# Da1yuqin/TCDiff

Measured on AMD Instinct MI355X. Metric: sampled clips/sec (3 dancers x 150 frames, 1000 DDPM steps), higher is better.
Workload: dtype bf16; 1 GPU; batch=16 clips/GPU, 3 dancers x 150 frames, 1000 DDPM steps (p_sample_loop, CFG w=2, cosine schedule), bf16, 1xMI355X; clips_per_gpu=16, ddpm_steps=1000

## Files before the change

### include/tcdiff_hip.h

```cpp
#ifndef TCDIFF_HIP_H
#define TCDIFF_HIP_H

#include <stdint.h>

#ifdef __cplusplus
extern "C" {
#endif

#ifndef __HIP__
typedef struct ihipStream_t* hipStream_t;
#endif

#define TCDIFF_OK 0
#define TCDIFF_ERR_ARG (-1)
#define TCDIFF_ERR_ALIGN (-2)
#define TCDIFF_ERR_LAUNCH (-3)
#define TCDIFF_ERR_UNSUPPORTED (-4)

#define TC_DTYPE_F32 0
#define TC_DTYPE_BF16 1
#define TC_DTYPE_BF16X3 2

#define TC_ACT_NONE 0
#define TC_ACT_RELU 1
// ... 130 lines not shown
    int film_ld;
    float ln_eps, n2_eps, n4_eps, nn_eps, scale_q;
    const float* filmb;
    const float* n3_g;
    const float* n3_b;
    const void* kf;
    const void* vf;
    int n_shared, nkt, Lk;
    int xres_rowmajor;
    int rope_rows;
    int dn;
    int mt;
    int out_ld;
    int nw;
    int seq_blocks;
    const void* sa_q;
    const void* sa_kf;
    const void* sa_vf;
    int sa_nkt;
    void* qf_out;
    void* kf_out;
    void* vf_out;
    int out_nkt;
} tcdiff_chain_args;

int tcdiff_chain(const tcdiff_chain_args* args, hipStream_t stream);

int tcdiff_chain_split(const tcdiff_chain_args* args, int part, const float* p_in, float* p_out, hipStream_t stream);

int tcdiff_pack_kv_frags(const void* Kc, const void* Vc, void* Kf, void* Vf, int n_slots, int H, int Lp, int nkt,
                         int key_lo, int key_hi, hipStream_t stream);

int tcdiff_attention(int dtype, const void* Q, const void* K, const void* V, void* O, int n_seq, int H, int Lq,
                     int Lk, int Lp_q, int Lp_k, int ldo, int n_shared, int ng, hipStream_t stream);

int tcdiff_ln_rot(int dtype, const float* x, int rows, const float* g, const float* b, float eps, void* h,
                  void* rot, float* y32, const float* rope, int pos_mod, int pos_base, hipStream_t stream);

int tcdiff_rope_table(const float* freqs, float* rope, int n_pos, hipStream_t stream);

int tcdiff_convert_pad(int dtype, const float* src, void* dst, int rows, int cols, int ld_dst, int rows_per_batch,
                       long batch_stride, long row_stride, hipStream_t stream);
int tcdiff_sinusoidal(int dtype, const int* times, int n, const float* freq, void* emb, hipStream_t stream);
int tcdiff_mean_pool(const float* x, float* out, int B, int S, int C, hipStream_t stream);
int tcdiff_add_act(int dtype, const float* a, const int* ia, const float* b, int n, int act, void* out,
                   float* out32, hipStream_t stream);
// ... 397 lines not shown
```

### tcdiff_amd/csrc/chain.hip

```cpp
#include "common.h"
#include "tcdiff_hip.h"

#include "chain_core.h"

#ifdef CH_ABLATE_ROWLAT
#define CH_RP_NEXT(rp, nt) do { } while (0)
#else
#define CH_RP_NEXT(rp, nt) rp_issue(rp, nt)
#endif

template <int HH, int MT, int NT, bool SELF = false>
DEVINL void cross_attention(const f32x4_t (&qacc)[NT][MT], const tcdiff_chain_args& a, int m0, int Mv, int lblk, char* abuf,
                            int wave, int lane) {
#ifdef CH_XATT_ONEPASS
    constexpr bool PARK = !SELF;
#else
    constexpr bool PARK = false;
#endif
    constexpr bool ONEPASS = SELF || PARK;
    constexpr int NPS = ONEPASS ? 1 : (MT == 4 ? 2 : 1), NML = ONEPASS ? MT : (MT == 1 ? 1 : 2);
    lane = fresh_v(lane);
    wave = fresh_s(wave) * (NT / 4) + HH;
    const int c = lane & 15, g = lane >> 4;
    const int M = Mv, L = a.L, nkt = SELF ? a.sa_nkt : a.nkt, Lk = SELF ? a.L : a.Lk;
    const float qs = a.scale_q * CH_LOG2E;
    u32x4 qf[MT][2];
// ... 159 lines not shown
                        pk.x = pack_bf2(o[dt][ml][0] * inv, o[dt][ml][1] * inv);
                        pk.y = pack_bf2(o[dt][ml][2] * inv, o[dt][ml][3] * inv);
                        *reinterpret_cast<uint2*>(abuf + wave * 8192 + act_wr_off(lane, dt) + mt * 2048) = pk;
                    }
                }
            }
        }
    }
}

#ifdef CH_STAMP
#ifndef CH_STAMP_BLOCK
#define CH_STAMP_BLOCK 0
#endif
#define CH_T(i) do { if (m0 == 64 * CH_STAMP_BLOCK && (threadIdx.x & 63) == 0 && (MODE == TC_CHAIN_B || MODE == TC_CHAIN_FULL)) \
        reinterpret_cast<unsigned long long*>(a.h_out)[(threadIdx.x >> 6) * 64 + (i)] = __builtin_amdgcn_s_memrealtime(); } while (0)
#define CH_TC(i) do { if (m0 == 64 * CH_STAMP_BLOCK && (threadIdx.x & 63) == 0 && (MODE == TC_CHAIN_B || MODE == TC_CHAIN_FULL)) \
        reinterpret_cast<unsigned long long*>(a.h_out)[(threadIdx.x >> 6) * 64 + (i)] = __builtin_amdgcn_s_memtime(); } while (0)
#else
#define CH_TC(i) do { } while (0)
#define CH_T(i) do { } while (0)
#endif

template <int MODE, int MT, int NT, int BRK>
DEVINL void chain_body(const tcdiff_chain_args& a) {
    constexpr int BR = BRK;
    constexpr int NW = ChW<NT>::NW, NTH = 64 * NW, RD = ChW<NT>::D;
    constexpr bool HAS_A = MODE == TC_CHAIN_A || MODE == TC_CHAIN_FULL || MODE == TC_CHAIN_FULL_LAST;
    constexpr bool FULL = MODE == TC_CHAIN_FULL || MODE == TC_CHAIN_FULL_LAST;
    constexpr bool LAST = MODE == TC_CHAIN_B_LAST || MODE == TC_CHAIN_FULL_LAST;
    constexpr bool FRONT = MODE == TC_CHAIN_FRONT;
    extern __shared__ __attribute__((aligned(16))) char smem[];
    const int tid = threadIdx.x, lane = tid & 63;
    const int wave = __builtin_amdgcn_readfirstlane(tid >> 6);
    const int c = lane & 15, g = lane >> 4;
    const int dn = FRONT ? a.dn : 1;
    const int dancer = FRONT ? (int)(blockIdx.x % (unsigned)dn) : 0;
    const int lblk = FRONT ? (int)(blockIdx.x / (unsigned)dn) : xcd_remap(blockIdx.x, gridDim.x);
    const bool seqcut = !FRONT && a.seq_blocks;
    const int nbs = seqcut ? (a.L + BR - 1) / BR : 1;
    const int bseq = seqcut ? lblk / nbs : 0, bis = seqcut ? lblk - bseq * nbs : 0;
    const int m0 = seqcut ? bseq * a.L + bis * BR : lblk * BR;
    CH_T(0);
    CH_TC(60);
    const int Mtot = a.M, L = a.L;
    const int M = seqcut ? (bseq + 1) * L : Mtot;
    char* abuf = smem + CH_ABUF;
// ... 80 lines not shown
            for (int kt = 0; kt < (FRONT ? 16 : 8); ++kt)
                stage_glds<16 * MT, NWL>(abuf + kt * 8192, reinterpret_cast<const char*>(a.A) + kt * TC_ROWB, FRONT ? 2048 : 1024, m0,
                                    M, a.a_mod, wave, lane);
        }
        ring_fill();
    }
    if (FRONT) {
        const float* const v[6] = {a.b3 + 512 * dancer, a.nn_g, a.nn_b, nullptr, nullptr, nullptr};
        store_consts(fetch_consts(nullptr, v));
    } else {
        const float* const v[6] = {nullptr, nullptr, a.n2_g, a.n2_b, nullptr, nullptr};
        store_consts(fetch_consts(a.film, v));
    }
    __builtin_amdgcn_s_waitcnt(0x0F70);
    __syncthreads();
    CH_T(1);


    float nmr[MT], rstd[MT];
    RowPipe<MT> rp;
    const long xrows = (long)Mtot * dn;
    const __amdgpu_buffer_rsrc_t xo = f32_buffer(a.xout, xrows * 512);
    Consts nxt;

    auto fc_epilogue = [&](float eps, int stamp) {
        CH_T(stamp);
        row_stats(acc, scr, wave, lane, eps, nmr, rstd);
        CH_T(stamp + 1);
        const int gg = fresh_v(g), wv = fresh_s(wave);
        const Rows rw = rows();
        const int cb0 = col_base_bytes<NT>(wv, gg);
        auto body = [&](int nt, int mt, const f32x4_t& G, const f32x4_t& Bv) {
            const f32x4_t x4 = rp.q[nt & 1][mt];
            f32x4_t o;
#pragma unroll
            for (int t = 0; t < 4; ++t) {
                float v = fmaf(fmaf(acc[nt][mt][t], rstd[mt], nmr[mt]), G[t], Bv[t]);
                v = x4[t] + v;
                acc[nt][mt][t] = v;
                o[t] = v;
            }
#ifdef CH_STORE_EARLY
            cb_store<NT>(xo, Mtot, wv, nt, rw.mc[mt], gg, o);
#endif
        };
        int fb[MT];
#pragma unroll
        for (int mt = 0; mt < MT; ++mt) {
            fb[mt] = rw.sidx[mt] * 4096 + cb0;
            asm volatile("" : "+v"(fb[mt]));
        }
#pragma unroll
        for (int nt = 0; nt < NT; ++nt) {
#pragma unroll
            for (int mt = 0; mt < MT; ++mt)
                body(nt, mt, lds4b(cfilm + fb[mt], 64 * nt), lds4b(cfilm + fb[mt], 2048 + 64 * nt));
            if (nt + 2 < NT) CH_RP_NEXT(rp, nt + 2);
            CH_FENCE();
        }
#ifndef CH_STORE_EARLY
#pragma unroll
        for (int nt = 0; nt < NT; ++nt)
#pragma unroll
            for (int mt = 0; mt < MT; ++mt) cb_store<NT>(xo, Mtot, wv, nt, rw.mc[mt], gg, acc[nt][mt]);
#endif
    };
    auto xres_start = [&]() {
        const Rows rw = rows();
        int rr[MT];
#pragma unroll
        for (int mt = 0; mt < MT; ++mt) rr[mt] = a.xres_mod > 0 ? rw.mc[mt] % a.xres_mod : rw.mc[mt];
        rp_start<NT>(rp, a.xres, rr, a.xres_rowmajor ? 0 : (a.xres_mod > 0 ? a.xres_mod : Mtot), a.xres_mod > 0 ? a.xres_mod : Mtot, wave,
                     fresh_v(g));
    };
    auto xout_start = [&]() {
        const Rows rw = rows();
        rp_start<NT>(rp, a.xout, rw.mc, Mtot, Mtot, wave, fresh_v(g));
    };
    auto rope_start = [&]() {
        const Rows rw = rows();
        int pos[MT];
        positions(rw, pos);
        rp_start<NT>(rp, a.rope, pos, a.rope_rows, a.rope_rows, wave, fresh_v(g));
    };

    if (HAS_A) {
        zero(acc);
        phase_n512<16, false, MT, NT>(acc, abuf, ws, lane);
        CH_T(2);
        xres_start();
        fc_epilogue(a.ln_eps, 40);
        CH_T(3);
        if (FULL) {
            const float* const v[6] = {nullptr, nullptr, n3_g, n3_b, nullptr, nullptr};
            nxt = fetch_consts(fcb_film, v);
        }
        rope_start();
        row_stats(acc, scr + 1024, wave, lane, a.n2_eps, nmr, rstd);
        CH_T(4);
        norm_to_lds<true, MT, NT>(acc, nmr, rstd, vecp(2), vecp(3), rp, abuf, wave, lane, nullptr);
        lds_barrier();
        CH_T(34);
        if (FULL) store_consts(nxt);
        zero(acc);
        if (!FULL) {
            phase_n512<16, false, MT, NT>(acc, abuf, ws, lane);
            store_heads<true, MT, NT>(acc, a.q_out, a.scale_q, L, a.Lp, a.H, m0, M, wave, lane, smem);
            return;
        }
#ifdef CH_STAMP
        {
            unsigned long long* sp = nullptr;
            if (m0 == 64 * CH_STAMP_BLOCK) {
                sp = reinterpret_cast<unsigned long long*>(a.h_out) + 512 + wave * 32;
                if (lane == 0) sp[16] = __builtin_amdgcn_s_memtime();
            }
            phase_n512<16, false, MT, NT>(acc, abuf, ws, lane, sp);
        }
#else
        phase_n512<16, false, MT, NT>(acc, abuf, ws, lane);
#endif
        CH_T(35);
        lds_barrier();
#ifndef CH_ABLATE_XATTN
        cross_attention<0>(acc, a, m0, M, lblk, abuf, wave, lane);
        if constexpr (NT == 8) cross_attention<1>(acc, a, m0, M, lblk, abuf, wave, lane);
#endif
        CH_T(36);
        lds_barrier();
    }
    if constexpr (!FRONT) {
    zero(acc);
    phase_n512<16, false, MT, NT>(acc, abuf, ws, lane);
    if (FULL)
        xout_start();
    else
        xres_start();
    CH_T(37);
    fc_epilogue(a.ln_eps, 42);
    CH_T(38);
    row_stats(acc, scr + 1024, wave, lane, a.n2_eps, nmr, rstd);
    CH_T(39);
    {
        const float* const v[6] = {a.b1, a.b1 + 512, nullptr, a.n4_g, a.n4_b, nullptr};
        nxt = fetch_consts(a.film3, v);
    }
    norm_to_lds<false, MT, NT>(acc, nmr, rstd, vecp(2), vecp(3), rp, abuf, wave, lane, nullptr);
    lds_barrier();
    store_consts(nxt);
    lds_barrier();
    CH_T(5);
    zero(acc);
#pragma unroll 1
    for (int ch = 0; ch < 4; ++ch) {
        f32x4_t a1[NT / 2][MT];
#pragma unroll
        for (int nt = 0; nt < NT / 2; ++nt)
#pragma unroll
            for (int mt = 0; mt < MT; ++mt) a1[nt][mt] = f32x4_t{0, 0, 0, 0};
        phase_ff1<MT, NT>(a1, abuf, ws, lane);
        CH_T(6 + 4 * ch);
        char* hb = h1c + (ch & 1) * 32768;
// ... 42 lines not shown
        }
#pragma unroll
        for (int nt = 0; nt < NT; ++nt) {
#pragma unroll
            for (int mt = 0; mt < MT; ++mt)
                body2(nt, mt, lds4b(cfilm + fb2[mt], 64 * nt), lds4b(cfilm + fb2[mt], 2048 + 64 * nt));
            if (nt + 2 < NT) CH_RP_NEXT(rp, nt + 2);
            CH_FENCE();
        }
    }
    CH_T(22);
    {
        const float* const v[6] = {a.b3, a.nn_g, a.nn_b, nullptr, nullptr, nullptr};
        nxt = fetch_consts(nullptr, v);
    }
    row_stats(acc, scr, wave, lane, a.n4_eps, nmr, rstd);
    CH_T(23);
    norm_to_lds<false, MT, NT>(acc, nmr, rstd, vecp(3), vecp(4), rp, abuf, wave, lane, nullptr);
    lds_barrier();
    store_consts(nxt);
    }
    CH_T(24);
    zero(acc);
    if (FRONT)
        phase_n512<32, false, MT, NT>(acc, abuf, ws, lane);
    else if (LAST)
        phase_n512<16, true, MT, NT>(acc, abuf, ws, lane);
    else
        phase_n512<16, false, MT, NT>(acc, abuf, ws, lane);
    CH_T(25);
    lds_barrier();
#ifndef CH_STORE_EARLY
    if (!LAST) rope_start();
#endif
    {
        const int g3 = fresh_v(g);
        const int cb3 = col_base_bytes<NT>(fresh_s(wave), g3);
        const Rows rw = rows();
#pragma unroll
        for (int nt = 0; nt < NT; ++nt) {
            const int n = 16 * NT * wave + 16 * nt + 4 * g3;
            const f32x4_t b4 = lds4b(vecp(0) + cb3, 64 * nt);
#pragma unroll
            for (int mt = 0; mt < MT; ++mt) {
                f32x4_t o;
#pragma unroll
                for (int t = 0; t < 4; ++t) {
                    acc[nt][mt][t] += b4[t];
                    o[t] = acc[nt][mt][t];
                }
                if (LAST && a.out_ld > 0) {
                    if (n < a.out_ld)
                        *reinterpret_cast<f32x4_t*>(reinterpret_cast<float*>(a.h_out) + (long)rw.mc[mt] * a.out_ld + n) = o;
                } else if (LAST) {
                    uint2 pk;
                    pk.x = pack_bf2(o[0], o[1]);
                    pk.y = pack_bf2(o[2], o[3]);
                    *reinterpret_cast<uint2*>(reinterpret_cast<uint16_t*>(a.h_out) + (long)rw.mc[mt] * 512 + n) = pk;
// ... 30 lines not shown
    if constexpr (FRAG) {
        if (frag_out) store_kfrag<MT>(acc, a.kf_out, bseq, bis * BR, a.out_nkt, wave, lane);
    }
    if (!frag_out) store_heads<false, MT, NT>(acc, a.k_out, 1.0f, L, a.Lp, a.H, m0, M, wave, lane, smem, dn, dancer);
    CH_T(31);
    zero(acc);
    if constexpr (FRAG) {
        if (frag_out) {
            phase_n512<16, true, MT, NT, true>(acc, smem + CH_ABUF2, ws, lane);
            CH_T(32);
            store_vfrag<MT>(acc, a.vf_out, bseq, bis * BR, a.out_nkt, L, wave, lane);
            CH_T(33);
            CH_TC(61);
            return;
        }
    }
    phase_n512<16, true, MT, NT>(acc, smem + CH_ABUF2, ws, lane);
    CH_T(32);
    store_heads<false, MT, NT>(acc, a.v_out, 1.0f, L, a.Lp, a.H, m0, M, wave, lane, smem, dn, dancer);
    CH_T(33);
    CH_TC(61);
}

template <int MODE, int MT, int NT>
__global__ __launch_bounds__(2048 / NT) void chain_kernel(tcdiff_chain_args a) {
    constexpr bool DUAL = (MODE == TC_CHAIN_FULL || MODE == TC_CHAIN_FULL_LAST) && NT == 4 && MT > 1;
    if constexpr (DUAL) {
        if (a.seq_blocks) {
            const int lblk = xcd_remap(blockIdx.x, gridDim.x);
            const int nbs = (a.L + 16 * MT - 1) / (16 * MT);
            if (a.L - (lblk % nbs) * 16 * MT <= 16) {
                chain_body<MODE, 1, NT, 16 * MT>(a);
                return;
            }
        }
    }
    chain_body<MODE, MT, NT, 16 * MT>(a);
}

static bool al16(const void* p) { return (reinterpret_cast<uintptr_t>(p) & 15) == 0; }

extern "C" int tcdiff_chain(const tcdiff_chain_args* a, hipStream_t stream) {
    if (!a || a->M <= 0 || a->L <= 0 || !a->A || !a->wstream) return TC_ERR_ARG;
    const bool front = a->mode == TC_CHAIN_FRONT;
    if (!front && a->L < 64) return TC_ERR_UNSUPPORTED;
    const int want = a->mode == TC_CHAIN_A ? 32 : a->mode == TC_CHAIN_B ? 144 : a->mode == TC_CHAIN_B_LAST ? 96 :
                     a->mode == TC_CHAIN_FULL ? 176 : a->mode == TC_CHAIN_FULL_LAST ? 128 : front ? 80 : -1;
    if (want < 0 || a->n_stages != want) return TC_ERR_ARG;
    if (a->out_ld < 0 || a->out_ld % 4 || a->out_ld > 512) return TC_ERR_ARG;
    const void* ptrs[] = {a->A, a->wstream, a->film, a->xres, a->xout, a->n2_g, a->n2_b, a->rope,
                          a->q_out, a->b1, a->film3, a->n4_g, a->n4_b, a->b3, a->nn_g, a->nn_b, a->k_out,
                          a->v_out, a->h_out, a->filmb, a->n3_g, a->n3_b, a->kf, a->vf};
    for (const void* p : ptrs)
        if (p && !al16(p)) return TC_ERR_ALIGN;
    if (front) {
        if (a->dn <= 0 || a->L % a->dn || a->L / a->dn < 8 || !a->b3 || !a->nn_g || !a->nn_b || !a->rope || !a->xout ||
            !a->q_out || !a->k_out || !a->v_out || a->H != 8 || a->Lp <= 0 || a->a_mod != 0)
            return TC_ERR_ARG;
        if ((long)a->M * 2048 >= (1L << 32)) return TC_ERR_ARG;
    } else {
// ... 8 lines not shown
    if (a->mode == TC_CHAIN_A && (!a->q_out || a->Lp <= 0)) return TC_ERR_ARG;
    if (has_b && (!a->b1 || !a->film3 || !a->n4_g || !a->n4_b || !a->b3)) return TC_ERR_ARG;
    const bool frag_out = a->qf_out || a->kf_out || a->vf_out;
    if (has_b && !last &&
        (!a->rope || !a->nn_g || !a->nn_b || (!frag_out && (!a->q_out || !a->k_out || !a->v_out)) || a->H != 8 || a->Lp <= 0))
        return TC_ERR_ARG;
    if (last && !a->h_out) return TC_ERR_ARG;
    if (full && (!a->filmb || !a->n3_g || !a->n3_b || !a->kf || !a->vf || a->nkt <= 0 ||
                 a->Lk <= 0 || a->Lk > 32 * a->nkt || a->n_shared < 0))
        return TC_ERR_ARG;
    if (a->seq_blocks && (front || a->M % a->L)) return TC_ERR_ARG;
    if (a->sa_q && (!full || !a->seq_blocks || !a->sa_kf || !a->sa_vf || a->sa_nkt <= 0 || a->L > 32 * a->sa_nkt)) return TC_ERR_ARG;
    if (frag_out && (!a->qf_out || !a->kf_out || !a->vf_out || !has_b || last || !a->seq_blocks || a->out_nkt <= 0 ||
                     a->L > 32 * a->out_nkt))
        return TC_ERR_ARG;
    if ((a->sa_q || frag_out) && a->nw == 4) return TC_ERR_UNSUPPORTED;
    for (const void* p : {a->sa_q, a->sa_kf, a->sa_vf, (const void*)a->qf_out, (const void*)a->kf_out, (const void*)a->vf_out})
        if (p && !al16(p)) return TC_ERR_ALIGN;
    if (a->sa_q && (long)(a->M / a->L) * 8 * a->sa_nkt * 4096 >= (1L << 32)) return TC_ERR_ARG;
    static tc_dev_state dev_state;
    const int n_cu = tc_device_once(dev_state, [](int) {
#define CH_FN(M_, NT_) reinterpret_cast<const void*>(chain_kernel<M_, 4, NT_>), reinterpret_cast<const void*>(chain_kernel<M_, 2, NT_>), \
                        reinterpret_cast<const void*>(chain_kernel<M_, 1, NT_>)
        const void* fns[27] = {CH_FN(TC_CHAIN_A, 4), CH_FN(TC_CHAIN_B, 4), CH_FN(TC_CHAIN_B_LAST, 4), CH_FN(TC_CHAIN_FULL, 4),
                               CH_FN(TC_CHAIN_FULL_LAST, 4), CH_FN(TC_CHAIN_FRONT, 4),
                               CH_FN(TC_CHAIN_FULL, 8), CH_FN(TC_CHAIN_FULL_LAST, 8), CH_FN(TC_CHAIN_FRONT, 8)};
#undef CH_FN
        for (const void* f : fns) {
            hipError_t e = hipFuncSetAttribute(f, hipFuncAttributeMaxDynamicSharedMemorySize, CH_SMEM);
            if (e != hipSuccess) return e;
        }
        return hipSuccess;
    });
    if (n_cu < 0) return n_cu;
    const int units = front ? a->dn : 1;
    int mt = a->mt;
    if (mt == 0) mt = ((a->M + 15) / 16) * units <= n_cu ? 1 : ((a->M + 31) / 32) * units <= n_cu ? 2 : 4;
    if (mt != 1 && mt != 2 && mt != 4) return TC_ERR_ARG;
    dim3 grid(((a->M + 16 * mt - 1) / (16 * mt)) * units);
    if (a->seq_blocks) grid.x = (a->M / a->L) * ((a->L + 16 * mt - 1) / (16 * mt));
    if (a->nw != 0 && a->nw != 4 && a->nw != 8) return TC_ERR_ARG;
    const bool four = a->nw == 4;
    if (four && !(full || front)) return TC_ERR_UNSUPPORTED;
#define CH_LAUNCH_NT(MODE_, NT_)                                                                                              \
    do {                                                                                                                      \
        if (mt == 4) hipLaunchKernelGGL((chain_kernel<MODE_, 4, NT_>), grid, dim3(2048 / NT_), CH_SMEM, stream, *a);          \
        else if (mt == 2) hipLaunchKernelGGL((chain_kernel<MODE_, 2, NT_>), grid, dim3(2048 / NT_), CH_SMEM, stream, *a);     \
        else hipLaunchKernelGGL((chain_kernel<MODE_, 1, NT_>), grid, dim3(2048 / NT_), CH_SMEM, stream, *a);                  \
    } while (0)
#define CH_LAUNCH(MODE_) CH_LAUNCH_NT(MODE_, 4)
#define CH_LAUNCH2(MODE_) do { if (four) CH_LAUNCH_NT(MODE_, 8); else CH_LAUNCH_NT(MODE_, 4); } while (0)
    switch (a->mode) {
        case TC_CHAIN_FRONT: CH_LAUNCH2(TC_CHAIN_FRONT); break;
        case TC_CHAIN_A: CH_LAUNCH(TC_CHAIN_A); break;
        case TC_CHAIN_B: CH_LAUNCH(TC_CHAIN_B); break;
        case TC_CHAIN_B_LAST: CH_LAUNCH(TC_CHAIN_B_LAST); break;
        case TC_CHAIN_FULL: CH_LAUNCH2(TC_CHAIN_FULL); break;
        default: CH_LAUNCH2(TC_CHAIN_FULL_LAST); break;
    }
#undef CH_LAUNCH
#undef CH_LAUNCH2
#undef CH_LAUNCH_NT
    TC_CHECK_LAUNCH();
    return TC_OK;
}
```

### tcdiff_amd/csrc/chain_core.h

```cpp
#pragma once
#include "common.h"
#include "tcdiff_hip.h"

#define CH_FILM 0
#define CH_VEC 8192
#define CH_SCR 20480
#define CH_ABUF 28672
#define CH_H1C 94208
#define CH_ABUF2 94208
#define CH_STG7 159744
#define CH_SMEM 163840
#define CH_D 4
#define CH_STAGE 4096
#ifndef CH_D8
#define CH_D8 4
#endif
template <int NT> struct ChW {
    static constexpr int NW = 32 / NT;
    static constexpr int D = NT == 8 ? CH_D8 : CH_D;
    static constexpr int STAGE = 1024 * NT;
};

typedef const float* fptr;

DEVINL void mma16(f32x4_t& acc, const u32x4& a, const u32x4& b) {
    acc = __builtin_amdgcn_mfma_f32_16x16x32_bf16(__builtin_bit_cast(bf16x8_t, a), __builtin_bit_cast(bf16x8_t, b), acc, 0, 0, 0);
}

template <int NT = 4>
struct WStreamT {
    __amdgpu_buffer_rsrc_t rsrc;
    unsigned voff;
    unsigned pos;
    unsigned last;
    u32x4 w[ChW<NT>::D][NT];
};
typedef WStreamT<4> WStream;
template <int NT>
DEVINL void ws_load(WStreamT<NT>& ws, int slot, unsigned stage) {
    const unsigned st = stage < ws.last ? stage : ws.last;
    const unsigned so = st * (unsigned)ChW<NT>::STAGE;
#pragma unroll
    for (int i = 0; i < NT; ++i)
        ws.w[slot][i] = __builtin_bit_cast(u32x4, __builtin_amdgcn_raw_buffer_load_b128(ws.rsrc, ws.voff + 1024u * i, so, 0));
}
#define CH_FENCE() do { asm volatile("" ::: "memory"); __builtin_amdgcn_sched_barrier(0); } while (0)
// ... 280 lines not shown
    return *reinterpret_cast<const f32x4_t*>(base + byte_off);
}
DEVINL f32x4_t lds4(const char* base, int float_index) {
    return *reinterpret_cast<const f32x4_t*>(base + float_index * 4);
}
template <int NT = 4>
DEVINL int col_base_bytes(int wave, int g) {
    int v = (16 * NT * wave + 4 * g) * 4;
    asm volatile("" : "+v"(v));
    return v;
}

template <int MT>
struct RowPipe {
    __amdgpu_buffer_rsrc_t rsrc;
    unsigned voff[MT];
    unsigned soff, its;
    f32x4_t q[2][MT];
};
DEVINL __amdgpu_buffer_rsrc_t f32_buffer(const float* base, long n_floats) {
    const long bytes = n_floats * 4;
    return __builtin_amdgcn_make_buffer_rsrc(const_cast<float*>(base), 0, bytes < 0xFFFFFFFFl ? (int)bytes : -1, 0x00020000);
}
template <int MT>
DEVINL void rp_issue(RowPipe<MT>& rp, int nt) {
#pragma unroll
    for (int mt = 0; mt < MT; ++mt)
        rp.q[nt & 1][mt] = __builtin_bit_cast(
            f32x4_t, __builtin_amdgcn_raw_buffer_load_b128(rp.rsrc, rp.voff[mt], rp.soff + (unsigned)nt * rp.its, 0));
}
template <int NT, int MT>
DEVINL void rp_start(RowPipe<MT>& rp, const float* base, const int (&row)[MT], long rows, long total_rows, int wave, int g) {
    rp.rsrc = f32_buffer(base, total_rows * 512);
    const unsigned grp = rows > 0 ? (unsigned)rows * 32u : 0u;
    rp.its = rows > 0 ? 2u * grp : 64u;
    rp.soff = rows > 0 ? (unsigned)wave * (2u * NT) * grp : (unsigned)wave * (64u * NT);
    const unsigned gterm = rows > 0 ? (unsigned)(g >> 1) * grp + 16u * (g & 1) : 16u * g;
#pragma unroll
    for (int mt = 0; mt < MT; ++mt)
        rp.voff[mt] = (rows > 0 ? (unsigned)row[mt] * 32u : (unsigned)row[mt] * 2048u) + gterm;
    rp_issue(rp, 0);
    rp_issue(rp, 1);
}
template <int NT = 4>
DEVINL void cb_store(__amdgpu_buffer_rsrc_t rsrc, long rows, int wave, int nt, int row, int g, f32x4_t v) {
    const unsigned grp = (unsigned)rows * 32u;
    __builtin_amdgcn_raw_buffer_store_b128(__builtin_bit_cast(u32x4, v), rsrc,
                                           (unsigned)row * 32u + (unsigned)(g >> 1) * grp + 16u * (g & 1),
                                           (unsigned)(wave * 2 * NT + 2 * nt) * grp, 0);
}

DEVINL int act_wr_off(int lane, int nt, int chunk0 = 0) {
    const int c = lane & 15, g = lane >> 4;
    return c * TC_ROWB + (((chunk0 + 2 * nt + (g >> 1)) ^ tile_swz(c)) << 4) + 8 * (g & 1);
}

template <bool ROT, int MT, int NT>
DEVINL void norm_to_lds(const f32x4_t (&acc)[NT][MT], const float (&nmr)[MT], const float (&rstd)[MT], const char* gv,
                        const char* bv, RowPipe<MT>& rp, char* abuf, int wave, int lane, char* plain) {
    lane = fresh_v(lane);
    wave = fresh_s(wave);
    const int g = lane >> 4;
    const int cb0 = col_base_bytes<NT>(wave, g);
#pragma unroll
    for (int nt = 0; nt < NT; ++nt) {
// ... 172 lines not shown
```

### tcdiff_amd/engine.py

```python
from __future__ import annotations

import math
import os
from typing import Dict, Optional

import torch

from . import _lib as L
from . import kernels as K
from .form import Form, resolve_form
from .step_graphs import StepGraphs

NL_FILM = 3


class DenoiserEngine:
    def __init__(self, cfg: dict, device: torch.device, compute: str = "bf16"):
        L.load()
        if device.type != "cuda":
            raise L.TcdiffError("DenoiserEngine needs a HIP device (cuda:N); there is no CPU fallback")
        self.cfg = dict(cfg)
        self.dev = device
        self.dt = K.dtype_id(compute)
        self.T = K.TORCH_DT[self.dt]
# ... 506 lines not shown
    def _layer_chained(self, l: int, form: Form, xcur: int, B: int, branches: int, film0, fld: int, n_shared: int, kv_slot0: int) -> int:
        dt, b, Lq, H = self.dt, self.b, self.Lseq, self.H
        Rs, nseq = B * Lq, branches * B
        frag0 = l == 0 and form.frag_front
        if l == 0 and not self.front:
            K.gemm_tile(dt, b["rot"], self.w["l0.qkv.w"], Rs, 1536, 512, A2=b["h"], split_n=1024, mode=L.EPI_QKV_HEADS,
                        out=b["Q"], out_k=b["K"], out_v=b["V"], scale_q=0.125, Lseq=Lq, Lp=self.Lp, H=H, n_q=512,
                        n_k=512)
        if not (form.fused_sa and l > 0) and not frag0:
            K.attention(dt, b["Q"], b["K"], b["V"], b["O"], B if l == 0 else nseq, H, Lq, Lq, self.Lp, self.Lp, 512)
        head, tail = self._head_args(l, Rs, film0, fld), self._tail_args(l, form, frag0, film0)
        x_in = self._layer_input(l, Rs, frag0, b["xa"])
        if not self.use_full:
            self._layer_chain_ab(l, nseq, film0, fld, n_shared, kv_slot0, head, tail, x_in)
            return xcur
        w, p = self.w, f"l{l}."
        cross = dict(filmb=film0[:, (l * 3 + 1) * 1024:], n3_g=w[p + "norm3.g"], n3_b=w[p + "norm3.b"], kf=b["Kf"][l, kv_slot0:],
                     vf=b["Vf"][l, kv_slot0:], n_shared=n_shared, nkt=self.nkt, Lk=self.S + 2)
        if form.split:
            return self._layer_split(l, form, xcur, Rs, nseq, {**head, **tail, **cross})
        self._layer_fused(l, nseq, {**head, **tail, **cross}, x_in)
        return xcur

    def _head_args(self, l: int, Rs: int, film0, fld: int) -> dict:
        w, p = self.w, f"l{l}."
        return dict(a_mod=Rs if l == 0 else 0, ln_eps=1e-6,
                    film=film0[:, (l * 3 + 0) * 1024:], film_ld=fld, n2_g=w[p + "norm2.g"], n2_b=w[p + "norm2.b"], n2_eps=1e-5,
                    rope=w["rope_cb"])

    def _layer_input(self, l: int, Rs: int, frag0: bool, x) -> dict:
        if l == 0:
            return dict(xres=self.b["xs"], xres_mod=Rs, xres_rowmajor=not self.front or frag0)
        return dict(xres=x, xres_mod=0, xres_rowmajor=False)

    def _tail_args(self, l: int, form: Form, frag0: bool, film0) -> dict:
        w, b, p = self.w, self.b, f"l{l}."
        last = l + 1 == self.NL
        nn = f"l{l + 1}.norm1."
        tail = dict(b1=w[p + "ff1.b"], film3=film0[:, (l * 3 + 2) * 1024:], n4_g=w[p + "norm4.g"],
                    n4_b=w[p + "norm4.b"], n4_eps=1e-5, b3=w[p + "l3out.b"] if last and self.fold_out else w[p + "l3.b"],
                    nn_g=None if last else w[nn + "g"], nn_b=None if last else w[nn + "b"], nn_eps=1e-5,
                    q_out=None if last else b["Q"], k_out=None if last else b["K"], v_out=None if last else b["V"],
                    h_out=(b["out"] if self.fold_out else b["h"]) if last else None,
                    out_ld=152 if last and self.fold_out else 0, scale_q=0.125, Lp=self.Lp, H=self.H)
        if form.fused_sa:
            tail.update(seq_blocks=True, mt=form.mt)
            if l > 0 or frag0:
                tail.update(sa_q=b["Qf"], sa_kf=b["sKf"][l & 1], sa_vf=b["sVf"][l & 1], sa_nkt=self.skt)
            if not last:
                tail.update(q_out=None, k_out=None, v_out=None, qf_out=b["Qf"], kf_out=b["sKf"][(l + 1) & 1],
                            vf_out=b["sVf"][(l + 1) & 1], out_nkt=self.skt)
        return tail

    def _layer_split(self, l: int, form: Form, xcur: int, Rs: int, nseq: int, args: dict) -> int:
        b, Lq = self.b, self.Lseq
        X, P = (b["xa"], b["xb"]), (b["P0"], b["P1"])
        o = 0 if l == 0 else xcur ^ 1
        frag0 = l == 0 and form.frag_front
        mode = L.CHAIN_FULL_LAST if l + 1 == self.NL else L.CHAIN_FULL
        launch = lambda part, **io: K.chain(mode, nseq * Lq, Lq, b["O"], self.w[f"l{l}.chainF"], split_part=part, **args, **io)
        x_in = self._layer_input(l, Rs, frag0, X[xcur])
        if form.merge12:
            launch(12, p_out=P[1], **x_in, xout=X[o])
        else:
            launch(1, p_out=P[0], **self._layer_input(l, Rs, frag0, b["xa"]), xout=b["xa"])
            launch(2, p_in=P[0], p_out=P[1], **x_in, xout=X[o])
        launch(3, p_in=P[1], p_out=P[0], xres=X[o], xout=X[o ^ 1])
        launch(4, p_in=P[0], xres=X[o ^ 1], xout=X[o])
        return o

    def _layer_fused(self, l: int, nseq: int, args: dict, x_in: dict):
        K.chain(L.CHAIN_FULL_LAST if l + 1 == self.NL else L.CHAIN_FULL, nseq * self.Lseq, self.Lseq, self.b["O"],
                self.w[f"l{l}.chainF"], **args, **x_in, xout=self.b["xa"])

# ... 11 lines not shown
```

### tcdiff_amd/kernels.py

```python
import ctypes as C

import torch

from . import _lib as L

TORCH_DT = {L.DT_F32: torch.float32, L.DT_BF16: torch.bfloat16, L.DT_BF16X3: torch.float32}


def dtype_id(name_or_dtype) -> int:
    if isinstance(name_or_dtype, str) and name_or_dtype == "bf16x3":
        return L.DT_BF16X3
    if name_or_dtype in ("bf16", torch.bfloat16, L.DT_BF16):
        return L.DT_BF16
    if name_or_dtype in ("f32", "fp32", torch.float32, L.DT_F32):
        return L.DT_F32
    if name_or_dtype == L.DT_BF16X3 and not isinstance(name_or_dtype, bool):
        return L.DT_BF16X3
    raise ValueError(f"unsupported compute dtype {name_or_dtype!r} (bf16, f32 or bf16x3)")


def k_tile(dt: int) -> int:
    return 64 if dt == L.DT_BF16 else 32


# ... 105 lines not shown
def gemm_rowln(dt, A, W, M, K, *, flags, lda=None, ldw=None, a_mod=0, bias=None, ln_g=None, ln_b=None, ln_eps=1e-6,
               film=None, film_ld=0, xres=None, xres_mod=0, xout=None, Lseq=1, nln_g=None, nln_b=None, nln_eps=1e-5,
               hout=None, rout=None, rope=None, out_mul=1, out_add=0, groups=1):
    lib = L.load()
    e = L.RowEpi(flags, _p(bias), _p(ln_g), _p(ln_b), ln_eps, _p(film), film_ld, _p(xres), xres_mod, _p(xout), Lseq,
                 _p(nln_g), _p(nln_b), nln_eps, _p(hout), _p(rout), _p(rope), out_mul, out_add, groups)
    rc = lib.tcdiff_gemm_rowln(dt, _p(A), _p(W), M, K, lda if lda else K, ldw if ldw else K, a_mod, C.byref(e),
                               stream())
    L.check(rc, "tcdiff_gemm_rowln")


def attention(dt, Q, K, V, O, n_seq, H, Lq, Lk, Lp_q, Lp_k, ldo, n_shared=0, ng=0):
    rc = L.load().tcdiff_attention(dt, _p(Q), _p(K), _p(V), _p(O), n_seq, H, Lq, Lk, Lp_q, Lp_k, ldo, n_shared, ng,
                                   stream())
    L.check(rc, "tcdiff_attention")


def chain(mode, M, Lseq, A, wstream, *, ln_eps=1e-6, film=None, film_ld=0, xres=None,
          xout=None, n2_g=None, n2_b=None, n2_eps=1e-5,
          rope=None, q_out=None, scale_q=0.125, Lp=0, H=8, a_mod=0, xres_mod=0, b1=None, film3=None, n4_g=None,
          n4_b=None, n4_eps=1e-5, b3=None, nn_g=None, nn_b=None, nn_eps=1e-5, k_out=None, v_out=None, h_out=None,
          filmb=None, n3_g=None, n3_b=None, kf=None, vf=None, n_shared=0, nkt=0, Lk=0,
          xres_rowmajor=False, out_ld=0, dn=1, mt=0, seq_blocks=False, sa_q=None, sa_kf=None, sa_vf=None, sa_nkt=0,
          qf_out=None, kf_out=None, vf_out=None, out_nkt=0, split_part=None, p_in=None, p_out=None):
    nw = wstream.shape[-3]
    if (nw, wstream.shape[-1]) not in ((8, 2048), (4, 4096)) or not wstream.is_contiguous():
        raise L.TcdiffError("weight stream must be contiguous [.., 8 waves, n_stages, 2048] or [.., 4 waves, n_stages, 4096] bf16, "
                            f"got {tuple(wstream.shape)}")
    n_stages = wstream.shape[-2]
    a = L.ChainArgs(mode, n_stages, M, Lseq, a_mod, xres_mod, H, Lp, _p(A), _p(wstream), _p(film),
                    _p(xres), _p(xout), _p(n2_g), _p(n2_b), _p(rope), _p(q_out), _p(b1), _p(film3), _p(n4_g),
                    _p(n4_b), _p(b3), _p(nn_g), _p(nn_b), _p(k_out), _p(v_out), _p(h_out), film_ld, ln_eps, n2_eps,
                    n4_eps, nn_eps, scale_q, _p(filmb), _p(n3_g), _p(n3_b), _p(kf), _p(vf), n_shared,
                    nkt, Lk, int(bool(xres_rowmajor)), 0 if rope is None else rope.shape[1], dn, mt, out_ld, nw,
                    int(bool(seq_blocks)), _p(sa_q), _p(sa_kf), _p(sa_vf), sa_nkt, _p(qf_out), _p(kf_out), _p(vf_out), out_nkt)
    if split_part is not None:
        L.check(L.load().tcdiff_chain_split(C.byref(a), split_part, _p(p_in), _p(p_out), stream()), "tcdiff_chain_split")
        return
    L.check(L.load().tcdiff_chain(C.byref(a), stream()), "tcdiff_chain")


def fold_film(film: torch.Tensor, g, b) -> torch.Tensor:
    sc1 = film[:, :512] + 1.0
    return torch.cat([sc1 if g is None else g * sc1, b * sc1 + film[:, 512:1024]], 1).contiguous()


def to_cb(x: torch.Tensor) -> torch.Tensor:
    rows = x.shape[0]
    return x.reshape(rows, 64, 8).permute(1, 0, 2).contiguous()


def from_cb(x: torch.Tensor, rows: int) -> torch.Tensor:
    return x.reshape(64, rows, 8).permute(1, 0, 2).reshape(rows, 512).contiguous()


def pack_kv_frags(Kc, Vc, Kf, Vf, n_slots, H, Lp, nkt, key_lo, key_hi):
    L.check(L.load().tcdiff_pack_kv_frags(_p(Kc), _p(Vc), _p(Kf), _p(Vf), n_slots, H, Lp, nkt, key_lo, key_hi, stream()),
            "tcdiff_pack_kv_frags")
# ... 544 lines not shown
```

Baseline: 14.86 clips/s.

## Keep half of residual x in LDS between fused-layer fc epilogues

In FULL chain launches (except the nt=8,mt=4 shape), the first fc epilogue now writes the low half of the updated residual tiles into an LDS region instead of global memory. The second epilogue reads those tiles back from LDS with a rotated tile order, so only the upper half is prefetched from global xout. A second change lets waves in FULL_LAST skip the final phase when their output columns lie beyond out_ld. This aims to cut global stores and loads of x and some idle MFMA work, at the cost of more template instances, LDS pressure, and a new res_mem flag that restores the old path.

```diff
diff --git a/include/tcdiff_hip.h b/include/tcdiff_hip.h
--- a/include/tcdiff_hip.h
+++ b/include/tcdiff_hip.h
@@ -176,6 +176,7 @@
     void* kf_out;
     void* vf_out;
     int out_nkt;
+    int res_mem;
 } tcdiff_chain_args;
 
 int tcdiff_chain(const tcdiff_chain_args* args, hipStream_t stream);
diff --git a/tcdiff_amd/csrc/chain.hip b/tcdiff_amd/csrc/chain.hip
--- a/tcdiff_amd/csrc/chain.hip
+++ b/tcdiff_amd/csrc/chain.hip
@@ -2,6 +2,10 @@
 #include "tcdiff_hip.h"
 
 #include "chain_core.h"
+
+#if defined(CH_XATT_ONEPASS) && !defined(CH_RES_MEM)
+#error "CH_XATT_ONEPASS parks Q in the GELU chunk buffers, where a FULL launch keeps half of x between its fc epilogues: build with -DCH_RES_MEM"
+#endif
 
 #ifdef CH_ABLATE_ROWLAT
 #define CH_RP_NEXT(rp, nt) do { } while (0)
@@ -207,7 +211,7 @@
 #define CH_T(i) do { } while (0)
 #endif
 
-template <int MODE, int MT, int NT, int BRK>
+template <int MODE, int MT, int NT, int BRK, bool XLDS>
 DEVINL void chain_body(const tcdiff_chain_args& a) {
     constexpr int BR = BRK;
     constexpr int NW = ChW<NT>::NW, NTH = 64 * NW, RD = ChW<NT>::D;
@@ -334,16 +338,32 @@
     const long xrows = (long)Mtot * dn;
     const __amdgpu_buffer_rsrc_t xo = f32_buffer(a.xout, xrows * 512);
     Consts nxt;
-
-    auto fc_epilogue = [&](float eps, int stamp) {
+#ifdef CH_RES_MEM
+    constexpr bool xlds = false;
+#else
+    constexpr bool xlds = XLDS && FULL;
+    static_assert(!XLDS || (FULL && !ch_plain_full(NT, MT)), "no such instance");
+#endif
+
+    auto fc_epilogue = [&](float eps, int stamp, auto hand) {
+        constexpr int HAND = decltype(hand)::v;
         CH_T(stamp);
         row_stats(acc, scr, wave, lane, eps, nmr, rstd);
         CH_T(stamp + 1);
         const int gg = fresh_v(g), wv = fresh_s(wave);
         const Rows rw = rows();
         const int cb0 = col_base_bytes<NT>(wv, gg);
-        auto body = [&](int nt, int mt, const f32x4_t& G, const f32x4_t& Bv) {
-            const f32x4_t x4 = rp.q[nt & 1][mt];
+        constexpr bool lds_out = HAND == 1 && xlds, lds_in = HAND == 2 && xlds;
+        typedef __attribute__((address_space(3))) f32x4_t lds_f32x4;
+        unsigned ximg = 0;
+        if constexpr (lds_out || lds_in) {
+            ximg = (unsigned)reinterpret_cast<uintptr_t>(smem + CH_H1C) + wv * (2048 * NT) + fresh_v(lane) * 16;
+            asm volatile("" : "+v"(ximg));
+        }
+        auto xtile = [&](int nt, int mt) -> lds_f32x4& {
+            return *reinterpret_cast<lds_f32x4*>((uintptr_t)(ximg + (unsigned)((nt * MT + mt) * 1024)));
+        };
+        auto body = [&](int nt, int mt, const f32x4_t& x4, const f32x4_t& G, const f32x4_t& Bv) {
             f32x4_t o;
 #pragma unroll
             for (int t = 0; t < 4; ++t) {
@@ -353,7 +373,10 @@
                 o[t] = v;
             }
 #ifdef CH_STORE_EARLY
-            cb_store<NT>(xo, Mtot, wv, nt, rw.mc[mt], gg, o);
+            if (HAND == 1 && nt < NT / 2 && lds_out)
+                xtile(nt, mt) = o;
+            else
+                cb_store<NT>(xo, Mtot, wv, nt, rw.mc[mt], gg, o);
 #endif
         };
         int fb[MT];
@@ -362,19 +385,39 @@
             fb[mt] = rw.sidx[mt] * 4096 + cb0;
             asm volatile("" : "+v"(fb[mt]));
         }
-#pragma unroll
-        for (int nt = 0; nt < NT; ++nt) {
-#pragma unroll
-            for (int mt = 0; mt < MT; ++mt)
-                body(nt, mt, lds4b(cfilm + fb[mt], 64 * nt), lds4b(cfilm + fb[mt], 2048 + 64 * nt));
-            if (nt + 2 < NT) CH_RP_NEXT(rp, nt + 2);
-            CH_FENCE();
-        }
+        auto tiles = [&](auto rot) {
+            constexpr bool ROT = decltype(rot)::v != 0;
+#pragma unroll
+            for (int i = 0; i < NT; ++i) {
+                const int nt = ROT ? (i + NT / 2) % NT : i;
+#pragma unroll
+                for (int mt = 0; mt < MT; ++mt)
+                    body(nt, mt, rp.q[i & 1][mt], lds4b(cfilm + fb[mt], 64 * nt), lds4b(cfilm + fb[mt], 2048 + 64 * nt));
+                if (ROT && i + 2 >= NT / 2) {
+                    if (i + 2 < NT) {
+#pragma unroll
+                        for (int mt = 0; mt < MT; ++mt)
+                            rp.q[i & 1][mt] = xtile(i + 2 - NT / 2, mt);
+                    }
+                } else if (i + 2 < NT) {
+                    CH_RP_NEXT(rp, ROT ? i + 2 + NT / 2 : i + 2);
+                }
+                CH_FENCE();
+            }
+        };
+        tiles(ChInt<lds_in ? 1 : 0>{});
 #ifndef CH_STORE_EARLY
-#pragma unroll
-        for (int nt = 0; nt < NT; ++nt)
-#pragma unroll
-            for (int mt = 0; mt < MT; ++mt) cb_store<NT>(xo, Mtot, wv, nt, rw.mc[mt], gg, acc[nt][mt]);
+        auto stores = [&](auto low) {
+            constexpr bool LOW = decltype(low)::v != 0;
+#pragma unroll
+            for (int nt = 0; nt < NT; ++nt)
+#pragma unroll
+                for (int mt = 0; mt < MT; ++mt) {
+                    if (LOW && nt < NT / 2) xtile(nt, mt) = acc[nt][mt];
+                    else cb_store<NT>(xo, Mtot, wv, nt, rw.mc[mt], gg, acc[nt][mt]);
+                }
+        };
+        stores(ChInt<lds_out ? 1 : 0>{});
 #endif
     };
     auto xres_start = [&]() {
@@ -385,9 +428,9 @@
         rp_start<NT>(rp, a.xres, rr, a.xres_rowmajor ? 0 : (a.xres_mod > 0 ? a.xres_mod : Mtot), a.xres_mod > 0 ? a.xres_mod : Mtot, wave,
                      fresh_v(g));
     };
-    auto xout_start = [&]() {
+    auto xout_start = [&](int first = 0) {
         const Rows rw = rows();
-        rp_start<NT>(rp, a.xout, rw.mc, Mtot, Mtot, wave, fresh_v(g));
+        rp_start<NT>(rp, a.xout, rw.mc, Mtot, Mtot, wave, fresh_v(g), first);
     };
     auto rope_start = [&]() {
         const Rows rw = rows();
@@ -401,7 +444,7 @@
         phase_n512<16, false, MT, NT>(acc, abuf, ws, lane);
         CH_T(2);
         xres_start();
-        fc_epilogue(a.ln_eps, 40);
+        fc_epilogue(a.ln_eps, 40, ChInt<FULL ? 1 : 0>{});
         CH_T(3);
         if (FULL) {
             const float* const v[6] = {nullptr, nullptr, n3_g, n3_b, nullptr, nullptr};
@@ -445,11 +488,11 @@
     zero(acc);
     phase_n512<16, false, MT, NT>(acc, abuf, ws, lane);
     if (FULL)
-        xout_start();
+        xout_start(xlds ? NT / 2 : 0);
     else
         xres_start();
     CH_T(37);
-    fc_epilogue(a.ln_eps, 42);
+    fc_epilogue(a.ln_eps, 42, ChInt<FULL ? 2 : 0>{});
     CH_T(38);
     row_stats(acc, scr + 1024, wave, lane, a.n2_eps, nmr, rstd);
     CH_T(39);
@@ -538,18 +581,22 @@
     }
     CH_T(24);
     zero(acc);
+    bool idle3 = false;
+#ifndef CH_NO_SKIP3
+    if constexpr (MODE == TC_CHAIN_FULL_LAST && !ch_plain_full(NT, MT)) idle3 = a.out_ld > 0 && 16 * NT * wave >= a.out_ld;
+#endif
     if (FRONT)
         phase_n512<32, false, MT, NT>(acc, abuf, ws, lane);
-    else if (LAST)
-        phase_n512<16, true, MT, NT>(acc, abuf, ws, lane);
-    else
+    else if (LAST) {
+        if (!idle3) phase_n512<16, true, MT, NT>(acc, abuf, ws, lane);
+    } else
         phase_n512<16, false, MT, NT>(acc, abuf, ws, lane);
     CH_T(25);
     lds_barrier();
 #ifndef CH_STORE_EARLY
     if (!LAST) rope_start();
 #endif
-    {
+    if (!idle3) {
         const int g3 = fresh_v(g);
         const int cb3 = col_base_bytes<NT>(fresh_s(wave), g3);
         const Rows rw = rows();
@@ -626,7 +673,7 @@
     CH_TC(61);
 }
 
-template <int MODE, int MT, int NT>
+template <int MODE, int MT, int NT, bool XLDS = false>
 __global__ __launch_bounds__(2048 / NT) void chain_kernel(tcdiff_chain_args a) {
     constexpr bool DUAL = (MODE == TC_CHAIN_FULL || MODE == TC_CHAIN_FULL_LAST) && NT == 4 && MT > 1;
     if constexpr (DUAL) {
@@ -634,12 +681,12 @@
             const int lblk = xcd_remap(blockIdx.x, gridDim.x);
             const int nbs = (a.L + 16 * MT - 1) / (16 * MT);
             if (a.L - (lblk % nbs) * 16 * MT <= 16) {
-                chain_body<MODE, 1, NT, 16 * MT>(a);
+                chain_body<MODE, 1, NT, 16 * MT, XLDS>(a);
                 return;
             }
         }
     }
-    chain_body<MODE, MT, NT, 16 * MT>(a);
+    chain_body<MODE, MT, NT, 16 * MT, XLDS>(a);
 }
 
 static bool al16(const void* p) { return (reinterpret_cast<uintptr_t>(p) & 15) == 0; }
@@ -694,10 +741,16 @@
     const int n_cu = tc_device_once(dev_state, [](int) {
 #define CH_FN(M_, NT_) reinterpret_cast<const void*>(chain_kernel<M_, 4, NT_>), reinterpret_cast<const void*>(chain_kernel<M_, 2, NT_>), \
                         reinterpret_cast<const void*>(chain_kernel<M_, 1, NT_>)
-        const void* fns[27] = {CH_FN(TC_CHAIN_A, 4), CH_FN(TC_CHAIN_B, 4), CH_FN(TC_CHAIN_B_LAST, 4), CH_FN(TC_CHAIN_FULL, 4),
+        static_assert(ch_plain_full(8, 4) && !ch_plain_full(8, 2) && !ch_plain_full(8, 1) && !ch_plain_full(4, 4), "CH_FNX, CH_LAUNCH2X");
+#define CH_FNX(M_) reinterpret_cast<const void*>(chain_kernel<M_, 4, 4, true>), reinterpret_cast<const void*>(chain_kernel<M_, 2, 4, true>), \
+                    reinterpret_cast<const void*>(chain_kernel<M_, 1, 4, true>), reinterpret_cast<const void*>(chain_kernel<M_, 2, 8, true>),   \
+                    reinterpret_cast<const void*>(chain_kernel<M_, 1, 8, true>)
+        const void* fns[37] = {CH_FN(TC_CHAIN_A, 4), CH_FN(TC_CHAIN_B, 4), CH_FN(TC_CHAIN_B_LAST, 4), CH_FN(TC_CHAIN_FULL, 4),
                                CH_FN(TC_CHAIN_FULL_LAST, 4), CH_FN(TC_CHAIN_FRONT, 4),
-                               CH_FN(TC_CHAIN_FULL, 8), CH_FN(TC_CHAIN_FULL_LAST, 8), CH_FN(TC_CHAIN_FRONT, 8)};
+                               CH_FN(TC_CHAIN_FULL, 8), CH_FN(TC_CHAIN_FULL_LAST, 8), CH_FN(TC_CHAIN_FRONT, 8),
+                               CH_FNX(TC_CHAIN_FULL), CH_FNX(TC_CHAIN_FULL_LAST)};
 #undef CH_FN
+#undef CH_FNX
         for (const void* f : fns) {
             hipError_t e = hipFuncSetAttribute(f, hipFuncAttributeMaxDynamicSharedMemorySize, CH_SMEM);
             if (e != hipSuccess) return e;
@@ -712,26 +765,35 @@
     dim3 grid(((a->M + 16 * mt - 1) / (16 * mt)) * units);
     if (a->seq_blocks) grid.x = (a->M / a->L) * ((a->L + 16 * mt - 1) / (16 * mt));
     if (a->nw != 0 && a->nw != 4 && a->nw != 8) return TC_ERR_ARG;
+    if (a->res_mem != 0 && a->res_mem != 1) return TC_ERR_ARG;
     const bool four = a->nw == 4;
     if (four && !(full || front)) return TC_ERR_UNSUPPORTED;
-#define CH_LAUNCH_NT(MODE_, NT_)                                                                                              \
+#define CH_LAUNCH_NT(MODE_, NT_, X_)                                                                                          \
     do {                                                                                                                      \
-        if (mt == 4) hipLaunchKernelGGL((chain_kernel<MODE_, 4, NT_>), grid, dim3(2048 / NT_), CH_SMEM, stream, *a);          \
-        else if (mt == 2) hipLaunchKernelGGL((chain_kernel<MODE_, 2, NT_>), grid, dim3(2048 / NT_), CH_SMEM, stream, *a);     \
-        else hipLaunchKernelGGL((chain_kernel<MODE_, 1, NT_>), grid, dim3(2048 / NT_), CH_SMEM, stream, *a);                  \
+        if (mt == 4) hipLaunchKernelGGL((chain_kernel<MODE_, 4, NT_, X_>), grid, dim3(2048 / NT_), CH_SMEM, stream, *a);      \
+        else if (mt == 2) hipLaunchKernelGGL((chain_kernel<MODE_, 2, NT_, X_>), grid, dim3(2048 / NT_), CH_SMEM, stream, *a); \
+        else hipLaunchKernelGGL((chain_kernel<MODE_, 1, NT_, X_>), grid, dim3(2048 / NT_), CH_SMEM, stream, *a);              \
     } while (0)
-#define CH_LAUNCH(MODE_) CH_LAUNCH_NT(MODE_, 4)
-#define CH_LAUNCH2(MODE_) do { if (four) CH_LAUNCH_NT(MODE_, 8); else CH_LAUNCH_NT(MODE_, 4); } while (0)
+#define CH_LAUNCH(MODE_) CH_LAUNCH_NT(MODE_, 4, false)
+#define CH_LAUNCH2(MODE_) do { if (four) CH_LAUNCH_NT(MODE_, 8, false); else CH_LAUNCH_NT(MODE_, 4, false); } while (0)
+#define CH_LAUNCH2X(MODE_)                                                                                                    \
+    do {                                                                                                                      \
+        if (a->res_mem || ch_plain_full(four ? 8 : 4, mt)) CH_LAUNCH2(MODE_);                                                 \
+        else if (!four) CH_LAUNCH_NT(MODE_, 4, true);                                                                         \
+        else if (mt == 2) hipLaunchKernelGGL((chain_kernel<MODE_, 2, 8, true>), grid, dim3(256), CH_SMEM, stream, *a);        \
+        else hipLaunchKernelGGL((chain_kernel<MODE_, 1, 8, true>), grid, dim3(256), CH_SMEM, stream, *a);                     \
+    } while (0)
     switch (a->mode) {
         case TC_CHAIN_FRONT: CH_LAUNCH2(TC_CHAIN_FRONT); break;
         case TC_CHAIN_A: CH_LAUNCH(TC_CHAIN_A); break;
         case TC_CHAIN_B: CH_LAUNCH(TC_CHAIN_B); break;
         case TC_CHAIN_B_LAST: CH_LAUNCH(TC_CHAIN_B_LAST); break;
-        case TC_CHAIN_FULL: CH_LAUNCH2(TC_CHAIN_FULL); break;
-        default: CH_LAUNCH2(TC_CHAIN_FULL_LAST); break;
+        case TC_CHAIN_FULL: CH_LAUNCH2X(TC_CHAIN_FULL); break;
+        default: CH_LAUNCH2X(TC_CHAIN_FULL_LAST); break;
     }
 #undef CH_LAUNCH
 #undef CH_LAUNCH2
+#undef CH_LAUNCH2X
 #undef CH_LAUNCH_NT
     TC_CHECK_LAUNCH();
     return TC_OK;
diff --git a/tcdiff_amd/csrc/chain_core.h b/tcdiff_amd/csrc/chain_core.h
--- a/tcdiff_amd/csrc/chain_core.h
+++ b/tcdiff_amd/csrc/chain_core.h
@@ -22,6 +22,8 @@
 };
 
 typedef const float* fptr;
+template <int V> struct ChInt { static constexpr int v = V; };
+constexpr bool ch_plain_full(int nt, int mt) { return nt == 8 && mt == 4; }
 
 DEVINL void mma16(f32x4_t& acc, const u32x4& a, const u32x4& b) {
     acc = __builtin_amdgcn_mfma_f32_16x16x32_bf16(__builtin_bit_cast(bf16x8_t, a), __builtin_bit_cast(bf16x8_t, b), acc, 0, 0, 0);
@@ -348,15 +350,21 @@
     const long bytes = n_floats * 4;
     return __builtin_amdgcn_make_buffer_rsrc(const_cast<float*>(base), 0, bytes < 0xFFFFFFFFl ? (int)bytes : -1, 0x00020000);
 }
+template <int SLOT, int MT>
+DEVINL void rp_issue_at(RowPipe<MT>& rp, int nt) {
+#pragma unroll
+    for (int mt = 0; mt < MT; ++mt)
+        rp.q[SLOT][mt] = __builtin_bit_cast(
+            f32x4_t, __builtin_amdgcn_raw_buffer_load_b128(rp.rsrc, rp.voff[mt], rp.soff + (unsigned)nt * rp.its, 0));
+}
 template <int MT>
 DEVINL void rp_issue(RowPipe<MT>& rp, int nt) {
-#pragma unroll
-    for (int mt = 0; mt < MT; ++mt)
-        rp.q[nt & 1][mt] = __builtin_bit_cast(
-            f32x4_t, __builtin_amdgcn_raw_buffer_load_b128(rp.rsrc, rp.voff[mt], rp.soff + (unsigned)nt * rp.its, 0));
+    if (nt & 1) rp_issue_at<1>(rp, nt);
+    else rp_issue_at<0>(rp, nt);
 }
 template <int NT, int MT>
-DEVINL void rp_start(RowPipe<MT>& rp, const float* base, const int (&row)[MT], long rows, long total_rows, int wave, int g) {
+DEVINL void rp_start(RowPipe<MT>& rp, const float* base, const int (&row)[MT], long rows, long total_rows, int wave, int g,
+                     int first = 0) {
     rp.rsrc = f32_buffer(base, total_rows * 512);
     const unsigned grp = rows > 0 ? (unsigned)rows * 32u : 0u;
     rp.its = rows > 0 ? 2u * grp : 64u;
@@ -365,8 +373,8 @@
 #pragma unroll
     for (int mt = 0; mt < MT; ++mt)
         rp.voff[mt] = (rows > 0 ? (unsigned)row[mt] * 32u : (unsigned)row[mt] * 2048u) + gterm;
-    rp_issue(rp, 0);
-    rp_issue(rp, 1);
+    rp_issue_at<0>(rp, first);
+    rp_issue_at<1>(rp, first + 1);
 }
 template <int NT = 4>
 DEVINL void cb_store(__amdgpu_buffer_rsrc_t rsrc, long rows, int wave, int nt, int row, int g, f32x4_t v) {
diff --git a/tcdiff_amd/engine.py b/tcdiff_amd/engine.py
--- a/tcdiff_amd/engine.py
+++ b/tcdiff_amd/engine.py
@@ -552,9 +552,10 @@
         self._layer_fused(l, nseq, {**head, **tail, **cross}, x_in)
         return xcur
 
-    def _head_args(self, l: int, Rs: int, film0, fld: int) -> dict:
+    def _head_args(self, l: int, Rs: int, film0, fld: int, *, res_mem: int = 0) -> dict:
         w, p = self.w, f"l{l}."
-        return dict(a_mod=Rs if l == 0 else 0, ln_eps=1e-6,
+        head = {"res_mem": res_mem} if res_mem else {}
+        return dict(**head, a_mod=Rs if l == 0 else 0, ln_eps=1e-6,
                     film=film0[:, (l * 3 + 0) * 1024:], film_ld=fld, n2_g=w[p + "norm2.g"], n2_b=w[p + "norm2.b"], n2_eps=1e-5,
                     rope=w["rope_cb"])
 
@@ -563,7 +564,7 @@
             return dict(xres=self.b["xs"], xres_mod=Rs, xres_rowmajor=not self.front or frag0)
         return dict(xres=x, xres_mod=0, xres_rowmajor=False)
 
-    def _tail_args(self, l: int, form: Form, frag0: bool, film0) -> dict:
+    def _tail_args(self, l: int, form: Form, frag0: bool, film0, *, res_mem: int = 0) -> dict:
         w, b, p = self.w, self.b, f"l{l}."
         last = l + 1 == self.NL
         nn = f"l{l + 1}.norm1."
@@ -580,6 +581,8 @@
             if not last:
                 tail.update(q_out=None, k_out=None, v_out=None, qf_out=b["Qf"], kf_out=b["sKf"][(l + 1) & 1],
                             vf_out=b["sVf"][(l + 1) & 1], out_nkt=self.skt)
+        if res_mem:
+            tail.update(res_mem=res_mem)
         return tail
 
     def _layer_split(self, l: int, form: Form, xcur: int, Rs: int, nseq: int, args: dict) -> int:
diff --git a/tcdiff_amd/kernels.py b/tcdiff_amd/kernels.py
--- a/tcdiff_amd/kernels.py
+++ b/tcdiff_amd/kernels.py
@@ -151,7 +151,7 @@
           n4_b=None, n4_eps=1e-5, b3=None, nn_g=None, nn_b=None, nn_eps=1e-5, k_out=None, v_out=None, h_out=None,
           filmb=None, n3_g=None, n3_b=None, kf=None, vf=None, n_shared=0, nkt=0, Lk=0,
           xres_rowmajor=False, out_ld=0, dn=1, mt=0, seq_blocks=False, sa_q=None, sa_kf=None, sa_vf=None, sa_nkt=0,
-          qf_out=None, kf_out=None, vf_out=None, out_nkt=0, split_part=None, p_in=None, p_out=None):
+          qf_out=None, kf_out=None, vf_out=None, out_nkt=0, split_part=None, p_in=None, p_out=None, res_mem=0):
     nw = wstream.shape[-3]
     if (nw, wstream.shape[-1]) not in ((8, 2048), (4, 4096)) or not wstream.is_contiguous():
         raise L.TcdiffError("weight stream must be contiguous [.., 8 waves, n_stages, 2048] or [.., 4 waves, n_stages, 4096] bf16, "
@@ -162,7 +162,8 @@
                     _p(n4_b), _p(b3), _p(nn_g), _p(nn_b), _p(k_out), _p(v_out), _p(h_out), film_ld, ln_eps, n2_eps,
                     n4_eps, nn_eps, scale_q, _p(filmb), _p(n3_g), _p(n3_b), _p(kf), _p(vf), n_shared,
                     nkt, Lk, int(bool(xres_rowmajor)), 0 if rope is None else rope.shape[1], dn, mt, out_ld, nw,
-                    int(bool(seq_blocks)), _p(sa_q), _p(sa_kf), _p(sa_vf), sa_nkt, _p(qf_out), _p(kf_out), _p(vf_out), out_nkt)
+                    int(bool(seq_blocks)), _p(sa_q), _p(sa_kf), _p(sa_vf), sa_nkt, _p(qf_out), _p(kf_out), _p(vf_out), out_nkt,
+                    int(res_mem))
     if split_part is not None:
         L.check(L.load().tcdiff_chain_split(C.byref(a), split_part, _p(p_in), _p(p_out), stream()), "tcdiff_chain_split")
         return
```

Result: faster. 15.04 clips/s, median of 6 (+1.2%).
